# OlegArenz/gmmvi

Measured on AMD Instinct MI355X. Metric: samples_components_per_sec, higher is better.
Workload: dtype f32; 1 GPU; ns: stm target D=20, K=100 components (100/GPU), 100 samples/component, N=10000 samples/iter, SAMTRON (Stein, fixed K, reuse ratio 0, KL trust regions, improvement-based stepsizes); K=100, D=20, N=10000, parallelism=component-shard x1

## Files before the change

### gmmvi_amd/_lib.py

```python
import ctypes as C
import os

_HERE = os.path.dirname(os.path.abspath(__file__))
LIB_PATH = os.environ.get("GMMVI_HIP_LIB", os.path.join(_HERE, "libgmmvi_hip.so"))

GAUSS, STUDENT_T = 0, 1
SELF_NORMALIZED, OWN_SAMPLES_ONLY, EXPLICIT_ESTIMATE = 1, 2, 4
MAX_DIM = 64
MORE_REGISTER_MAX_DIM = 21
MORE_BLOCKED_MIN_DIM, MORE_BLOCKED_MAX_DIM = 64, 128
MAX_DIM_BLOCKED = 512
MAX_DIM_DIAG = 131072
BLOCKED_ABOVE_DEFAULT = 50


_blocked_above = None


def _atoi(text):
    import re
    m = re.match(r"\s*([+-]?\d+)", text)
    return int(m.group(1)) if m else 0


# ... 61 lines not shown
    "gmmvi_cholesky": (_i, [_p, _i, _i, _p, _p, _p]),
    "gmmvi_mixture_eval": (_i, [_p, _i, _f, _i, _i, _p, _p, _p, _i, _p, _p, _p]),
    "gmmvi_mixture_eval_dual": (_i, [_p, _i, _f, _i, _i, _p, _p, _p, _p, _i, _p, _p, _p, _p]),
    "gmmvi_target_planar": (_i, [_p, _i, _p, _i, _p, _f, _p, _i, _p, _p]),
    "gmmvi_target_logreg": (_i, [_p, _i, _i, _p, _f, _f, _p, _i, _p, _p]),
    "gmmvi_target_logreg_mb": (_i, [_p, _i, _i, _p, _i, _i, _u64, _u32, _f, _f, _p, _i, _p, _p]),
    "gmmvi_target_bnn": (_i, [_p, _i, _i, _i, _i, _p, _p, _u64, _u32, _i, _f, _f, _p, _i, _p, _p]),
    "gmmvi_bnn_predict": (_i, [_p, _i, _i, _i, _p, _i, _p, _i, _p]),
    "gmmvi_target_talos": (_i, [_p, _p, _p, _p, _i, _p, _p]),
    "gmmvi_talos_fk": (_i, [_p, _p, _p, _i, _p, _p]),
    "gmmvi_sample_components": (_i, [_p, _i, _i, _p, _p, _p, _i, _u64, _u64, _i, _p, _p, _p]),
    "gmmvi_philox_normals": (_i, [_p, _u64, _u64, _i, _i, _i, _p]),
    "gmmvi_philox_uniforms": (_i, [_p, _u64, _u64, _i, _i, _p]),
    "gmmvi_stein": (_i, [_p, _i, _i, _p, _p, _i, _p, _p, _p, _p, _p, _i, _i, _p, _p]),
    "gmmvi_more": (_i, [_p, _i, _i, _p, _p, _p, _i, _p, _p, _p, _p, _p, _i, _i, _p, _p, _p]),
    "gmmvi_more_blocked": (_i, [_p, _i, _i, _p, _p, _p, _i, _p, _p, _p, _p, _p, _i, _i, _p, _p, _p]),
    "gmmvi_update_components_kl": (_i, [_p, _i, _i, _p, _p, _p, _p, _p, _f, _f, _p, _p, _p, _p, _p, _p, _p]),
    "gmmvi_update_components_kl_reference": (_i, [_p, _i, _i, _p, _p, _p, _p, _p, _f, _f, _p, _p, _p, _p, _p, _p]),
    "gmmvi_update_components_direct": (_i, [_p, _i, _i, _p, _p, _p, _p, _p, _f, _p, _p, _p]),
    "gmmvi_update_components_iblr": (_i, [_p, _i, _i, _p, _p, _p, _p, _p, _f, _p, _p, _p]),
    "gmmvi_expected_log_ratios": (_i, [_p, _i, _i, _p, _p, _p, _p, _f, _p, _i, _p, _p, _p]),
    "gmmvi_update_weights_kl": (_i, [_p, _i, _p, _p, _p, _f, _p]),
    "gmmvi_update_weights_direct": (_i, [_p, _i, _p, _p, _p, _f]),
    "gmmvi_component_stepsize_improvement": (_i, [_p, _i, _p, _p, _p, _f, _f, _f, _f]),
    "gmmvi_weight_stepsize_improvement": (_i, [_p, _i, _p, _p, _p, _f, _f, _f, _f]),
    "gmmvi_train_iter_samtron": (_i, [_p, _p]),
    "gmmvi_sharded_scratch_floats": (_sz, [_i, _i, _i]),
    "gmmvi_train_iter_sharded_phase": (_i, [_p, _p, _i]),
    "gmmvi_comm_unique_id": (_i, [C.c_char_p]),
    "gmmvi_comm_init": (_i, [_p, C.c_char_p, _i, _i]),
    "gmmvi_comm_destroy": (_i, [_p]),
    "gmmvi_allgather_f32": (_i, [_p, _p, _p, _sz]),
    "gmmvi_allreduce_f32": (_i, [_p, _p, _sz, _i]),
    "gmmvi_combine_partials": (_i, [_p, _i, _i, _i, _p, _p, _p, _p]),
    "gmmvi_diag_packed_stride": (_sz, [_i]),
    "gmmvi_diag_pack": (_i, [_p, _i, _i, _p, _p, _p]),
    "gmmvi_diag_mixture_eval": (_i, [_p, _i, _i, _p, _p, _p, _p, _i, _p, _p, _p, _p]),
    "gmmvi_diag_sample": (_i, [_p, _i, _i, _p, _p, _p, _i, _u64, _u64, _i, _p, _p, _p]),
    "gmmvi_diag_stein": (_i, [_p, _i, _i, _p, _p, _i, _p, _p, _p, _p, _p, _i, _i, _p, _p]),
    "gmmvi_diag_embed": (_i, [_p, _i, _i, _p, _p]),
    "gmmvi_diag_extract": (_i, [_p, _i, _i, _p, _p]),
    "gmmvi_reciprocal_f32": (_i, [_p, _p, _sz, _p]),
    "gmmvi_update_components_diag_kl": (_i, [_p, _i, _i, _p, _p, _p, _p, _p, _f, _f, _p, _p, _p, _p, _p, _p]),
    "gmmvi_update_components_diag_iblr": (_i, [_p, _i, _i, _p, _p, _p, _p, _p, _f, _p, _p, _p]),
    "gmmvi_mmd_scratch_doubles": (_sz, [_i, _i]),
    "gmmvi_mmd_pair_sum": (_i, [_p, _p, _i, _p, _i, _i, _p, _p, _p]),
# ... 31 lines not shown
```

### gmmvi_amd/csrc/api.hip

```cpp
#include "common.h"
#include <cstring>
#include "blocked.h"

std::string g_gmmvi_global_err;

int gmmvi_ws_reserve(gmmvi_ctx* ctx, size_t nbytes) {
    ++ctx->ws_epoch;
    if (nbytes <= ctx->ws_bytes) return GMMVI_OK;
    GMMVI_HIP_CHECK(ctx, hipStreamSynchronize(ctx->stream));
    if (ctx->ws) GMMVI_HIP_CHECK(ctx, hipFree(ctx->ws));
    ctx->ws = nullptr;
    ctx->ws_bytes = 0;
    size_t want = nbytes + nbytes / 2;
    GMMVI_HIP_CHECK(ctx, hipMalloc(&ctx->ws, want));
    ctx->ws_bytes = want;
    return GMMVI_OK;
}

extern "C" {

int gmmvi_device_count(void) {
    int n = 0;
    if (hipGetDeviceCount(&n) != hipSuccess) return 0;
    return n;
}

int gmmvi_ctx_create(gmmvi_ctx** out, int device) {
    if (!out) return gmmvi_fail(nullptr, GMMVI_ERR_ARG, "gmmvi_ctx_create: out is NULL");
    *out = nullptr;
    int n = 0;
    hipError_t e = hipGetDeviceCount(&n);
    if (e != hipSuccess || n == 0)
        return gmmvi_fail(nullptr, GMMVI_ERR_HIP, std::string("no HIP device: ") + hipGetErrorString(e));
    if (device < 0 || device >= n) return gmmvi_fail(nullptr, GMMVI_ERR_ARG, "device index out of range");
    gmmvi_ctx* ctx = new gmmvi_ctx();
    ctx->device = device;
    e = hipSetDevice(device);
    if (e == hipSuccess) e = hipStreamCreateWithFlags(&ctx->stream, hipStreamNonBlocking);
    if (e != hipSuccess) {
        g_gmmvi_global_err = std::string("gmmvi_ctx_create: ") + hipGetErrorString(e);
        delete ctx;
        return GMMVI_ERR_HIP;
    }
    hipDeviceProp_t prop;
    if (hipGetDeviceProperties(&prop, device) == hipSuccess) ctx->num_cus = prop.multiProcessorCount;
    *out = ctx;
    return GMMVI_OK;
}

void gmmvi_ctx_destroy(gmmvi_ctx* ctx) {
    if (!ctx) return;
    gmmvi_comm_destroy(ctx);
    if (ctx->stream) {
        (void)hipStreamSynchronize(ctx->stream);
        (void)hipStreamDestroy(ctx->stream);
    }
    if (ctx->ws) (void)hipFree(ctx->ws);
    if (ctx->arena) (void)hipFree(ctx->arena);
    if (ctx->bimg) (void)hipFree(ctx->bimg);
    if (ctx->up_ring) {
        for (int i = 0; i < gmmvi_ctx::UP_SLOTS; ++i) (void)hipEventDestroy(ctx->up_event[i]);
        (void)hipHostFree(ctx->up_ring);
    }
    if (ctx->defer_ws) (void)hipFree(ctx->defer_ws);
    delete ctx;
}

const char* gmmvi_last_error(gmmvi_ctx* ctx) { return ctx ? ctx->err.c_str() : g_gmmvi_global_err.c_str(); }

int gmmvi_sync(gmmvi_ctx* ctx) {
    GMMVI_HIP_CHECK(ctx, hipStreamSynchronize(ctx->stream));
    return GMMVI_OK;
}

int gmmvi_malloc(gmmvi_ctx* ctx, size_t nbytes, void** out_dev) {
    GMMVI_ARG_CHECK(ctx, out_dev != nullptr);
    *out_dev = nullptr;
    if (nbytes == 0) nbytes = 4;
    GMMVI_HIP_CHECK(ctx, hipSetDevice(ctx->device));
    GMMVI_HIP_CHECK(ctx, hipMalloc(out_dev, nbytes));
    return GMMVI_OK;
}

int gmmvi_free(gmmvi_ctx* ctx, void* dev) {
    if (!dev) return GMMVI_OK;
    GMMVI_HIP_CHECK(ctx, hipFree(dev));
    return GMMVI_OK;
// ... 488 lines not shown
```

### gmmvi_amd/csrc/common.h

```cpp
#pragma once
#include <hip/hip_runtime.h>
#include <cstdio>
#include <cstring>
#include <cstdint>
#include <string>
#include <vector>
#include "../../include/gmmvi_hip.h"
#include "iter_prep.h"

struct CombineJob {
    int R = 0, N = 0, D = 0;
    long part_stride = 0;
    int first_block = 0, blocks = 0;
    const float* lp_parts = nullptr;
    const float* grad_parts = nullptr;
    const float* lp2_parts = nullptr;
    float* lp_out = nullptr;
    float* grad_out = nullptr;
    float* lp2_out = nullptr;
};

struct SampleJob {
    int K = 0, D = 0, uniform_count = 0;
    const float* means = nullptr; const float* chols = nullptr; const int32_t* offsets = nullptr;
// ... 14 lines not shown
}

struct gmmvi_ctx {
    int device = 0;
    hipStream_t stream = nullptr;
    std::string err;
    void* ws = nullptr;
    size_t ws_bytes = 0;
    uint64_t ws_epoch = 0;
    void* arena = nullptr;
    size_t arena_bytes = 0;
    static constexpr int UP_SLOTS = 64;
    static constexpr size_t UP_SLOT_BYTES = 64 * 1024;
    unsigned char* up_ring = nullptr;
    hipEvent_t up_event[UP_SLOTS] = {};
    bool up_used[UP_SLOTS] = {};
    int up_next = 0;
    void* bimg = nullptr;
    size_t bimg_bytes = 0;
    bool defer_combine = false;
    CombineJob pending;
    Riders riders;
    void* defer_ws = nullptr;
    size_t defer_bytes = 0;
    void* comm = nullptr;
    int n_ranks = 1, rank = 0;
    int num_cus = 256;
    unsigned func_attr_done = 0;
    bool prof = false;
    const char* prof_tag = nullptr;
    struct ProfRec { const char* name; hipEvent_t start, stop; double units; };
    std::vector<ProfRec> prof_recs;
};

struct GmmviProfScope {
    gmmvi_ctx* ctx; hipEvent_t stop = nullptr;
    GmmviProfScope(gmmvi_ctx* c, const char* name, double units = 0.0) : ctx(c) {
        if (!c->prof) return;
        hipEvent_t start;
        if (hipEventCreate(&start) != hipSuccess || hipEventCreate(&stop) != hipSuccess) { stop = nullptr; return; }
        (void)hipEventRecord(start, c->stream);
        c->prof_recs.push_back({name, start, stop, units});
    }
    ~GmmviProfScope() { if (stop) (void)hipEventRecord(stop, ctx->stream); }
};
#define GMMVI_PROF(ctx, name) GmmviProfScope prof_scope__(ctx, name)
// ... 33 lines not shown
int gmmvi_sample_components_prep(gmmvi_ctx* ctx, int K, int D, const float* means_dev, const float* chols_dev,
                                 const int32_t* offsets_dev, int N, int max_per_component, uint64_t seed, uint64_t first_index,
                                 float* X_out_dev, int32_t* mapping_out_dev, int32_t mapping_base, const PrepArgs& prep);
int gmmvi_combine_partials_internal(gmmvi_ctx* ctx, int R, int N, int D, const float* lp_parts_dev,
                                    const float* grad_parts_dev, float* lp_out_dev, float* grad_out_dev,
                                    const float* lp2_parts_dev, float* lp2_out_dev, long part_stride = 0);
int gmmvi_defer_reserve(gmmvi_ctx* ctx, size_t nbytes);
int gmmvi_flush_pending_combine(gmmvi_ctx* ctx);
CombineJob gmmvi_take_pending_combine(gmmvi_ctx* ctx, int threads, int first_block, bool light = false);
Riders gmmvi_take_pending_riders(gmmvi_ctx* ctx, int first_block, int threads, bool prep_only = false);
int gmmvi_flush_pending_riders(gmmvi_ctx* ctx);
struct SteinSlab;
int gmmvi_stein_partials(gmmvi_ctx* ctx, int K, int D, const float* packed_dev, const float* X_dev, int N, const float* ld_dev,
                         const float* qgrad_dev, const float* bg_dev, const float* tgrad_dev, int flags, SteinSlab* slab);
int gmmvi_stein_finalize_slab(gmmvi_ctx* ctx, int K, int D, const SteinSlab& slab, int N, int flags, const float* packed_dev,
                              float* H_neg_out_dev, float* g_neg_out_dev);
int gmmvi_update_components_kl_from_slab(gmmvi_ctx* ctx, int K, int D, const SteinSlab& slab, int N, int stein_flags,
                                         const float* packed_old_dev, float* H_neg_dev, float* g_neg_dev, float* means_dev,
                                         float* chols_dev, const float* stepsizes_dev, float temperature, float l2_init,
                                         float* last_eta_dev, float* l2_dev, float* num_received_updates_dev,
                                         int32_t* success_out_dev, float* packed_out_dev);
int gmmvi_update_weights_internal(gmmvi_ctx* ctx, int mode, int K, float* logw_dev, const float* E_dev,
                                  const float* stepsize_dev, float beta, float* kl_eta_out_dev, float* exp_out_dev);

inline int gmmvi_padded_dim(int D) {
    static const int dps[] = {2, 4, 8, 10, 12, 16, 20, 24, 32, 40, 50, 64};
    for (int dp : dps) if (D <= dp) return dp;
    return -1;
}

#define GMMVI_DISPATCH_DP(DPVAL, ...)                  \
    switch (DPVAL) {                                   \
        case 2:  { constexpr int DP = 2;  __VA_ARGS__; } break;  \
        case 4:  { constexpr int DP = 4;  __VA_ARGS__; } break;  \
        case 8:  { constexpr int DP = 8;  __VA_ARGS__; } break;  \
        case 10: { constexpr int DP = 10; __VA_ARGS__; } break;  \
        case 12: { constexpr int DP = 12; __VA_ARGS__; } break;  \
        case 16: { constexpr int DP = 16; __VA_ARGS__; } break;  \
        case 20: { constexpr int DP = 20; __VA_ARGS__; } break;  \
        case 24: { constexpr int DP = 24; __VA_ARGS__; } break;  \
        case 32: { constexpr int DP = 32; __VA_ARGS__; } break;  \
        case 40: { constexpr int DP = 40; __VA_ARGS__; } break;  \
        case 50: { constexpr int DP = 50; __VA_ARGS__; } break;  \
        case 64: { constexpr int DP = 64; __VA_ARGS__; } break;  \
        default: return gmmvi_fail(ctx, GMMVI_ERR_ARG, "unsupported dimension (D must be <= 64)"); \
    }
// ... 95 lines not shown
```

### gmmvi_amd/csrc/fused.hip

```cpp
#include "common.h"
#include "stepsize_rules.h"
#include "iter_prep.h"
#include "stein_finalize.h"

namespace {
struct Arena {
    float *ld, *lq, *qgrad, *bg, *H, *g, *E;
    int32_t *mapping, *success;
};

}

static int arena_reserve(gmmvi_ctx* ctx, size_t floats) {
    if (floats * sizeof(float) <= ctx->arena_bytes) return GMMVI_OK;
    GMMVI_HIP_CHECK(ctx, hipStreamSynchronize(ctx->stream));
    if (ctx->arena) GMMVI_HIP_CHECK(ctx, hipFree(ctx->arena));
    ctx->arena = nullptr;
    ctx->arena_bytes = 0;
    size_t want = floats * sizeof(float) * 3 / 2;
    GMMVI_HIP_CHECK(ctx, hipMalloc(&ctx->arena, want));
    ctx->arena_bytes = want;
    return GMMVI_OK;
}

#define GMMVI_TRY(call)                \
    do {                               \
        int rc__ = (call);             \
        if (rc__ != GMMVI_OK) return rc__; \
    } while (0)

static int train_iter_samtron_body(gmmvi_ctx* ctx, const gmmvi_samtron_plan* p);

extern "C" int gmmvi_train_iter_samtron(gmmvi_ctx* ctx, const gmmvi_samtron_plan* p) {
    GMMVI_ARG_CHECK(ctx, ctx != nullptr);
    int rc = gmmvi_flush_pending_combine(ctx);
    if (rc == GMMVI_OK) rc = train_iter_samtron_body(ctx, p);
    if (rc != GMMVI_OK) {
        ctx->pending = CombineJob();
        ctx->riders.prep_blocks = ctx->riders.sample_blocks = 0;
        ctx->defer_combine = false;
        ctx->prof_tag = nullptr;
    }
    return rc;
}

static int train_iter_samtron_body(gmmvi_ctx* ctx, const gmmvi_samtron_plan* p) {
    GMMVI_ARG_CHECK(ctx, p != nullptr);
    GMMVI_ARG_CHECK(ctx, (p->target_kind >= 0 && p->target_kind <= 2) || p->target_kind == 4);
    GMMVI_ARG_CHECK(ctx, p->target_kind != 2 || (p->logreg_A && p->logreg_M >= 1 && p->logreg_prior_std > 0.f));
    GMMVI_ARG_CHECK(ctx, p->target_kind != 4 || (p->talos_model && p->talos_context && p->D == 34));
    const int K = p->K, D = p->D, N = p->N;
    GMMVI_ARG_CHECK(ctx, K >= 1 && D >= 1 && D < GMMVI_MAX_DIM && N >= 1);
    GMMVI_ARG_CHECK(ctx, p->means && p->chols && p->logw && p->packed && p->packed_new && p->stepsizes && p->last_eta &&
                             p->l2 && p->num_updates && p->offsets && p->bg_logw && p->db_samples && p->db_tlp &&
                             p->db_tgrad && p->db_mapping && p->reward_next && p->wstate);
    GMMVI_ARG_CHECK(ctx, p->n_old >= 0 && p->max_per_component >= 0 && p->phase >= 0 && p->phase <= 2);
    GMMVI_ARG_CHECK(ctx, p->n_old == 0 || (p->bg_packed != nullptr && p->bg_K >= 1 && p->bg_old != nullptr && p->bg_logw_new != nullptr));
    const int n_old = p->n_old;
    const int Na = n_old + N;
    const size_t KN = (size_t)K * Na, ND = (size_t)Na * D;
    const size_t floats = KN + 4 * (size_t)Na + ND + (size_t)K * D * D + (size_t)K * D + 3 * (size_t)K + Na + 64;
    GMMVI_TRY(arena_reserve(ctx, floats));
    Arena a;
    float* base = (float*)ctx->arena;
// ... 87 lines not shown
    GMMVI_TRY(gmmvi_flush_pending_riders(ctx));
    SteinSlab slab{nullptr, nullptr, 0};
    GMMVI_TRY(gmmvi_stein_partials(ctx, K, D, p->packed, xa, Na, a.ld, a.qgrad, a.bg, tgrad_a, p->stein_flags, &slab));
    GMMVI_TRY(gmmvi_update_components_kl_from_slab(ctx, K, D, slab, Na, p->stein_flags, p->packed, a.H, a.g, p->means, p->chols,
                                                   p->stepsizes, p->temperature, p->l2_init, p->last_eta, p->l2, p->num_updates,
                                                   p->success_out ? p->success_out : a.success, p->packed_new));
    }
    if (phase == 1) return GMMVI_OK;
    ctx->defer_combine = true;
    ctx->prof_tag = "sweep_post";
    int rc_post = gmmvi_mixture_eval(ctx, GMMVI_GAUSS, 0.f, K, D, p->packed_new, p->logw, xa, Na, a.ld, a.lq, nullptr);
    ctx->defer_combine = false;
    ctx->prof_tag = nullptr;
    GMMVI_TRY(rc_post);
    if (p->presample_next && n_old == 0) {
        const int max_pc = p->max_per_component > 0 ? p->max_per_component : (N + K - 1) / K;
        SampleJob& sj = ctx->riders.sample;
        sj.K = K; sj.D = D; sj.uniform_count = (long)K * max_pc == N ? max_pc : 0;
        sj.means = p->means; sj.chols = p->chols; sj.offsets = p->offsets;
        sj.seed = p->seed; sj.first_index = p->first_index + (uint64_t)N;
        sj.X = x + (size_t)N * D; sj.mapping = p->db_mapping + N; sj.mapping_base = p->mapping_base + K;
        ctx->riders.sample_blocks = K * ((max_pc + 255) / 256);
    }
    GMMVI_TRY(gmmvi_expected_log_ratios(ctx, K, Na, a.ld, a.bg, tlp_a, a.lq, p->temperature, p->logw,
                                        (p->stein_flags & GMMVI_SELF_NORMALIZED) ? 1 : 0, a.E, p->reward_next, nullptr));
    GMMVI_TRY(gmmvi_flush_pending_riders(ctx));
    if (K > 1) {
        GMMVI_TRY(gmmvi_update_weights_internal(ctx, p->weight_update_mode == 0 ? 0 : 1, K, p->logw, a.E, p->wstate,
                                                p->temperature, nullptr, p->weight_slot));
    }
    return GMMVI_OK;
}


namespace {
struct ShardArena { float *ld, *lq, *bg, *qgrad, *H, *g, *E; int32_t* success; };
}
extern "C" size_t gmmvi_sharded_scratch_floats(int K, int D, int N) {
    if (K < 1 || D < 1 || N < 1) return 0;
    return (size_t)K * N + 2 * (size_t)N + (size_t)N * D + (size_t)K * D * D + (size_t)K * D + 2 * (size_t)K + 64;
}
static void shard_arena(float* base, int K, int D, int N, ShardArena& a) {
    a.ld = base; base += (size_t)K * N;
    a.lq = base; base += N;
    a.bg = base; base += N;
    a.qgrad = base; base += (size_t)N * D;
    a.H = base; base += (size_t)K * D * D;
    a.g = base; base += (size_t)K * D;
    a.E = base; base += K;
    a.success = (int32_t*)base;
}

static int sharded_phase_body(gmmvi_ctx* ctx, const gmmvi_sharded_plan* p, int phase) {
// ... 133 lines not shown
```

### gmmvi_amd/csrc/weights.hip

```cpp
#include "common.h"
#include "riders.h"
#include "stepsize_rules.h"
#include "wave_reduce.h"
#include "combine.h"
#include <cfloat>

namespace {

__device__ __forceinline__ float wsum(float v) { return gmmvi_wave_sum(v); }
__device__ __forceinline__ float wmax(float v) { return gmmvi_wave_max(v); }

__device__ float block_max(float v, float* red) {
    v = wmax(v);
    __syncthreads();
    if ((threadIdx.x & 63) == 0) red[threadIdx.x >> 6] = v;
    __syncthreads();
    return fmaxf(fmaxf(red[0], red[1]), fmaxf(red[2], red[3]));
}
__device__ float block_sum(float v, float* red) {
    v = wsum(v);
    __syncthreads();
    if ((threadIdx.x & 63) == 0) red[threadIdx.x >> 6] = v;
    __syncthreads();
    return (red[0] + red[1]) + (red[2] + red[3]);
}

template <int R>
// ... 8 lines not shown
            const int n = min(n0 + 1024 * u, N - 1);
            av[u] = row[n] - bg[n];
            float lq;
            if constexpr (R == 0) lq = logq[n];
            else if constexpr (R > 0) lq = combine_log_values_n<R>(logq, N, n);
            else lq = combine_log_values(logq, Rrt, N, n);
            rv[u] = tlp[n] - beta * lq;
        }
#pragma unroll
        for (int u = 0; u < B; ++u) {
            if (n0 + 1024 * u < N) {
                const float a = av[u], rho = rv[u];
                const float mn = fmaxf(m, a);
                const float sc = __expf(m - mn), e = __expf(a - mn);
                s = fmaf(s, sc, e);
                se = fmaf(se, sc, e * rho);
                s2 = fmaf(s2, sc * sc, e * e);
                m = mn;
            }
        }
    }
}

__device__ __forceinline__ void elr_body(int N, const float* __restrict__ ld, const float* __restrict__ bg,
                                         const float* __restrict__ tlp, const float* __restrict__ logq, int logq_R,
                                         float beta, const float* __restrict__ logw, int self_normalized,
                                         float* __restrict__ E_out, float* __restrict__ reward_out,
                                         float* __restrict__ ess_out) {
    __shared__ float red[4][16];
    const int k = blockIdx.x;
    const float* row = ld + (size_t)k * N;
    float m = -3.0e38f, s = 0.f, se = 0.f, s2 = 0.f;
    switch (logq_R) {
        case 0: elr_accumulate<0>(N, row, bg, tlp, logq, 0, beta, m, s, se, s2); break;
        case 2: elr_accumulate<2>(N, row, bg, tlp, logq, 2, beta, m, s, se, s2); break;
        case 3: elr_accumulate<3>(N, row, bg, tlp, logq, 3, beta, m, s, se, s2); break;
        case 4: elr_accumulate<4>(N, row, bg, tlp, logq, 4, beta, m, s, se, s2); break;
        case 5: elr_accumulate<5>(N, row, bg, tlp, logq, 5, beta, m, s, se, s2); break;
        case 6: elr_accumulate<6>(N, row, bg, tlp, logq, 6, beta, m, s, se, s2); break;
        case 7: elr_accumulate<7>(N, row, bg, tlp, logq, 7, beta, m, s, se, s2); break;
        case 8: elr_accumulate<8>(N, row, bg, tlp, logq, 8, beta, m, s, se, s2); break;
        case 10: elr_accumulate<10>(N, row, bg, tlp, logq, 10, beta, m, s, se, s2); break;
        case 12: elr_accumulate<12>(N, row, bg, tlp, logq, 12, beta, m, s, se, s2); break;
        case 16: elr_accumulate<16>(N, row, bg, tlp, logq, 16, beta, m, s, se, s2); break;
        default: elr_accumulate<-1>(N, row, bg, tlp, logq, logq_R, beta, m, s, se, s2); break;
    }
    const float mw = wmax(m);
    const float f = __expf(m - mw);
    s = wsum(s * f); se = wsum(se * f); s2 = wsum(s2 * f * f);
    const int lane = threadIdx.x & 63, wave = threadIdx.x >> 6;
    if (lane == 0) { red[0][wave] = mw; red[1][wave] = s; red[2][wave] = se; red[3][wave] = s2; }
    __syncthreads();
    if (threadIdx.x == 0) {
        float M = -3.0e38f;
        for (int w = 0; w < 16; ++w) M = fmaxf(M, red[0][w]);
        float S = 0.f, SE = 0.f, S2 = 0.f;
        for (int w = 0; w < 16; ++w) {
            const float g = __expf(red[0][w] - M);
            S = fmaf(red[1][w], g, S); SE = fmaf(red[2][w], g, SE); S2 = fmaf(red[3][w], g * g, S2);
        }
        const float E = self_normalized ? SE / S : SE * __expf(M) / (float)N;
        if (E_out) E_out[k] = E;
        if (reward_out) reward_out[k] = beta * logw[k] + E;
        if (ess_out) ess_out[k] = (S * S) / S2;
    }
}

__global__ __launch_bounds__(1024) void elr_kernel(int N, const float* __restrict__ ld, const float* __restrict__ bg,
                                                   const float* __restrict__ tlp, const float* __restrict__ logq, int logq_R,
                                                   float beta, const float* __restrict__ logw, int self_normalized,
                                                   float* __restrict__ E_out, float* __restrict__ reward_out,
                                                   float* __restrict__ ess_out) {
    elr_body(N, ld, bg, tlp, logq, logq_R, beta, logw, self_normalized, E_out, reward_out, ess_out);
}

template <int DP>
__global__ __launch_bounds__(1024) void elr_riders_kernel(int N, const float* __restrict__ ld, const float* __restrict__ bg,
                                                          const float* __restrict__ tlp, const float* __restrict__ logq,
                                                          int logq_R, float beta, const float* __restrict__ logw,
                                                          int self_normalized, float* __restrict__ E_out,
                                                          float* __restrict__ reward_out, float* __restrict__ ess_out,
                                                          Riders riders) {
    extern __shared__ __align__(16) float sm_riders[];
    if (riders_carried<DP>(riders, sm_riders)) return;
    elr_body(N, ld, bg, tlp, logq, logq_R, beta, logw, self_normalized, E_out, reward_out, ess_out);
}

__device__ float wave_lse(const float* v, int K) {
// ... 77 lines not shown
    bool ub_ok = false;
    for (int it = 0; it < 50; ++it) {
        eta = expf(log_eta);
        if (fabsf(expf(ub) - expf(lb)) < 1e-1f) break;
        kl = weights_kl_reg<NE>(eta, beta, lw, E, h, v);
        if (fabsf(bound - kl) < 1e-1f * bound) { lb = ub; break; }
        if (bound > kl) { ub = log_eta; ub_ok = true; } else { lb = log_eta; }
        log_eta = 0.5f * (ub + lb);
    }
    if (lb == ub) {
    } else if (ub_ok) {
        eta = expf(ub);
        kl = weights_kl_reg<NE>(eta, beta, lw, E, h, v);
    } else {
        updated = false;
        kl = -1.f; eta = -1.f;
    }
#pragma unroll
    for (int e = 0; e < NE; ++e)
        if (h[e]) nl[t + 64 * e] = v[e];
    __syncthreads();
}

__global__ __launch_bounds__(64) void update_weights_kernel(int mode, int K, float* __restrict__ logw,
                                                            const float* __restrict__ E_in, const float* __restrict__ stepsize,
                                                            float beta, float* __restrict__ kl_eta_out,
                                                            float* __restrict__ exp_out) {
    extern __shared__ float sm[];
    float* lw = sm; float* E = sm + K; float* nl = sm + 2 * K;
    const int t = threadIdx.x;
    for (int i = t; i < K; i += 64) { lw[i] = logw[i]; E[i] = E_in[i]; nl[i] = logw[i]; }
    __syncthreads();
    if (K <= 1) return;
    const float bound = stepsize[0];
    float kl = -1.f, eta = -1.f;
    bool updated = true;
    if (mode == 1) {
        for (int i = t; i < K; i += 64) nl[i] = lw[i] + bound / beta * E[i];
        __syncthreads();
        float l = wave_lse(nl, K);
        for (int i = t; i < K; i += 64) nl[i] = fmaxf(nl[i] - l, -69.07f);
        __syncthreads();
        l = wave_lse(nl, K);
        for (int i = t; i < K; i += 64) nl[i] -= l;
        __syncthreads();
    } else {
        if (K <= 128) {
            weights_search_reg<2>(K, beta, bound, lw, E, nl, kl, eta, updated);
        } else if (K <= 256) {
            weights_search_reg<4>(K, beta, bound, lw, E, nl, kl, eta, updated);
        } else if (K <= 512) {
            weights_search_reg<8>(K, beta, bound, lw, E, nl, kl, eta, updated);
        } else if (K <= 1024) {
            weights_search_reg<16>(K, beta, bound, lw, E, nl, kl, eta, updated);
// ... 12 lines not shown
            if (lb == ub) {
            } else if (ub_ok) {
                eta = expf(ub);
                kl = weights_kl(eta, beta, lw, E, nl, K);
            } else {
                updated = false;
                kl = -1.f; eta = -1.f;
            }
        }
    }
    if (!updated) {
        for (int i = t; i < K; i += 64) nl[i] = lw[i];
        __syncthreads();
    }
    const float l = wave_lse(nl, K);
    for (int i = t; i < K; i += 64) {
        const float v = nl[i] - l;
        logw[i] = v;
        if (exp_out) exp_out[i] = expf(v);
    }
    if (t == 0 && kl_eta_out) { kl_eta_out[0] = kl; kl_eta_out[1] = eta; }
}

__global__ void component_stepsize_kernel(int K, float* __restrict__ stepsizes, const float* __restrict__ prev,
                                          const float* __restrict__ last, float mn, float mx, float inc, float dec) {
    const int k = blockIdx.x * blockDim.x + threadIdx.x;
    if (k >= K) return;
    stepsizes[k] = component_stepsize_rule(stepsizes[k], prev[k], last[k], mn, mx, inc, dec);
}

__global__ __launch_bounds__(64) void weight_stepsize_kernel(int K, const float* __restrict__ logw,
                                                             const float* __restrict__ rewards_last, float* __restrict__ state,
                                                             float mn, float mx, float inc, float dec) {
    weight_stepsize_wave(K, logw, rewards_last, state, mn, mx, inc, dec, threadIdx.x);
}

}

extern "C" {

int gmmvi_expected_log_ratios(gmmvi_ctx* ctx, int K, int N, const float* ld_dev, const float* bg_dev,
                              const float* tlp_dev, const float* logq_dev, float beta, const float* logw_dev,
                              int self_normalized, float* E_out_dev, float* reward_out_dev, float* ess_out_dev) {
    GMMVI_ARG_CHECK(ctx, K >= 1 && N >= 1);
    GMMVI_ARG_CHECK(ctx, ld_dev && bg_dev && tlp_dev && logq_dev && logw_dev);
    int logq_R = 0;
    {
        const CombineJob& j = ctx->pending;
        if (j.R > 0 && j.lp_out == logq_dev && j.N == N && !j.grad_out && !j.lp2_out) {
            logq_R = j.R;
            logq_dev = j.lp_parts;
            ctx->pending = CombineJob();
        } else {
            int rc = gmmvi_flush_pending_combine(ctx);
            if (rc != GMMVI_OK) return rc;
        }
    }
    GMMVI_PROF(ctx, "expected_log_ratios");
    const Riders riders = gmmvi_take_pending_riders(ctx, K, 1024);
    if (riders.prep_blocks + riders.sample_blocks > 0) {
        const int dp = gmmvi_padded_dim(riders.sample_blocks > 0 ? riders.sample.D : 2);
        GMMVI_DISPATCH_DP(dp, hipLaunchKernelGGL((elr_riders_kernel<DP>), dim3(K + riders.prep_blocks + riders.sample_blocks),
                                                 dim3(1024), riders_lds_bytes(riders), ctx->stream, N, ld_dev, bg_dev, tlp_dev,
                                                 logq_dev, logq_R, beta, logw_dev, self_normalized, E_out_dev, reward_out_dev,
                                                 ess_out_dev, riders));
    } else {
        hipLaunchKernelGGL(elr_kernel, dim3(K), dim3(1024), 0, ctx->stream, N, ld_dev, bg_dev, tlp_dev, logq_dev, logq_R, beta,
                           logw_dev, self_normalized, E_out_dev, reward_out_dev, ess_out_dev);
    }
    GMMVI_LAUNCH_CHECK(ctx);
    return GMMVI_OK;
}

}

int gmmvi_update_weights_internal(gmmvi_ctx* ctx, int mode, int K, float* logw_dev, const float* E_dev,
                                  const float* stepsize_dev, float beta, float* kl_eta_out_dev, float* exp_out_dev) {
    GMMVI_ARG_CHECK(ctx, K >= 1 && K <= 4096);
    GMMVI_ARG_CHECK(ctx, logw_dev && E_dev && stepsize_dev);
    GMMVI_PROF(ctx, "update_weights");
    hipLaunchKernelGGL(update_weights_kernel, dim3(1), dim3(64), (size_t)3 * K * sizeof(float), ctx->stream, mode, K,
                       logw_dev, E_dev, stepsize_dev, beta, kl_eta_out_dev, exp_out_dev);
    GMMVI_LAUNCH_CHECK(ctx);
    return GMMVI_OK;
}

extern "C" {

int gmmvi_update_weights_kl(gmmvi_ctx* ctx, int K, float* logw_dev, const float* E_dev, const float* stepsize_dev,
                            float beta, float* kl_eta_out_dev) {
    return gmmvi_update_weights_internal(ctx, 0, K, logw_dev, E_dev, stepsize_dev, beta, kl_eta_out_dev, nullptr);
}

int gmmvi_update_weights_direct(gmmvi_ctx* ctx, int K, float* logw_dev, const float* E_dev,
                                const float* stepsize_dev, float beta) {
    return gmmvi_update_weights_internal(ctx, 1, K, logw_dev, E_dev, stepsize_dev, beta, nullptr, nullptr);
}

int gmmvi_component_stepsize_improvement(gmmvi_ctx* ctx, int K, float* stepsizes_dev, const float* rewards_prev_dev,
                                         const float* rewards_last_dev, float min_stepsize, float max_stepsize,
                                         float inc_factor, float dec_factor) {
    GMMVI_ARG_CHECK(ctx, K >= 1 && stepsizes_dev && rewards_prev_dev && rewards_last_dev);
    GMMVI_PROF(ctx, "component_stepsize");
    hipLaunchKernelGGL(component_stepsize_kernel, dim3((K + 127) / 128), dim3(128), 0, ctx->stream, K, stepsizes_dev,
                       rewards_prev_dev, rewards_last_dev, min_stepsize, max_stepsize, inc_factor, dec_factor);
    GMMVI_LAUNCH_CHECK(ctx);
    return GMMVI_OK;
}

int gmmvi_weight_stepsize_improvement(gmmvi_ctx* ctx, int K, const float* logw_dev, const float* rewards_last_dev,
// ... 12 lines not shown
```

### gmmvi_amd/hip_ops.py

```python
import math

import numpy as np

from . import _lib
from .device import DeviceArray

F32, I32 = np.dtype(np.float32), np.dtype(np.int32)


def _req(a, shape, dtype=F32, name="array"):
    if not isinstance(a, DeviceArray):
        raise TypeError(f"{name}: expected DeviceArray, got {type(a)}")
    if a.dtype != dtype or tuple(a.shape) != tuple(shape):
        raise ValueError(f"{name}: expected {dtype}{tuple(shape)}, got {a.dtype}{a.shape}")
    return a.ptr


def _opt(a, shape, dtype=F32, name="array"):
    return None if a is None else _req(a, shape, dtype, name)


def packed_stride(d):
    s = int(_lib.load().gmmvi_packed_stride(int(d)))
    if s == 0:
# ... 415 lines not shown
    if reward_out is not None:
        _req(reward_out, (k,), name="reward_out")
    e = ctx.empty((k,))
    ess = ctx.empty((k,)) if want_ess else None
    ctx.check(ctx.lib.gmmvi_expected_log_ratios(ctx.handle, k, n, ld.ptr, bg.ptr, tlp.ptr, logq.ptr, float(beta),
                                                logw.ptr, 1 if self_normalized else 0, e.ptr,
                                                None if reward_out is None else reward_out.ptr,
                                                None if ess is None else ess.ptr))
    return e, ess


def update_weights(ctx, mode, logw, e, stepsize, beta, want_info=False):
    k = logw.shape[0]
    _req(logw, (k,), name="logw"); _req(e, (k,), name="E"); _req(stepsize, (1,), name="stepsize")
    info = ctx.empty((2,)) if (want_info and mode == "trust-region") else None
    if mode == "trust-region":
        ctx.check(ctx.lib.gmmvi_update_weights_kl(ctx.handle, k, logw.ptr, e.ptr, stepsize.ptr, float(beta),
                                                  None if info is None else info.ptr))
    else:
        ctx.check(ctx.lib.gmmvi_update_weights_direct(ctx.handle, k, logw.ptr, e.ptr, stepsize.ptr, float(beta)))
    return info


def component_stepsize_improvement(ctx, stepsizes, prev, last, mn, mx, inc, dec):
    k = stepsizes.shape[0]
    _req(stepsizes, (k,), name="stepsizes"); _req(prev, (k,), name="prev"); _req(last, (k,), name="last")
    ctx.check(ctx.lib.gmmvi_component_stepsize_improvement(ctx.handle, k, stepsizes.ptr, prev.ptr, last.ptr, float(mn),
                                                           float(mx), float(inc), float(dec)))


def weight_stepsize_improvement(ctx, logw, rewards_last, state, mn, mx, inc, dec):
    k = logw.shape[0]
    _req(logw, (k,), name="logw"); _req(rewards_last, (k,), name="rewards_last"); _req(state, (2,), name="state")
    ctx.check(ctx.lib.gmmvi_weight_stepsize_improvement(ctx.handle, k, logw.ptr, rewards_last.ptr, state.ptr, float(mn),
                                                        float(mx), float(inc), float(dec)))


def combine_partials(ctx, lp_parts, grad_parts, d):
    r, n = lp_parts.shape
    _req(lp_parts, (r, n), name="lp_parts")
    if grad_parts is not None:
        _req(grad_parts, (r, n, d), name="grad_parts")
    lp = ctx.empty((n,))
    grad = ctx.empty((n, d)) if grad_parts is not None else None
    ctx.check(ctx.lib.gmmvi_combine_partials(ctx.handle, r, n, d, lp_parts.ptr,
                                             None if grad_parts is None else grad_parts.ptr, lp.ptr,
# ... 91 lines not shown
```

### include/gmmvi_hip.h

```cpp
#ifndef GMMVI_HIP_H
#define GMMVI_HIP_H

#include <stddef.h>
#include <stdint.h>

#ifdef __cplusplus
extern "C" {
#endif

typedef struct gmmvi_ctx gmmvi_ctx;

enum gmmvi_status {
    GMMVI_OK = 0,
    GMMVI_ERR_HIP = -1,
    GMMVI_ERR_ARG = -2,
    GMMVI_ERR_RCCL = -3,
    GMMVI_ERR_STATE = -4
};

enum gmmvi_family {
    GMMVI_GAUSS = 0,
    GMMVI_STUDENT_T = 1
};

// ... 117 lines not shown
                               float* num_received_updates_dev, int32_t* success_out_dev, float* kl_out_dev,
                               int32_t* n_probes_out_dev, float* packed_out_dev);
int gmmvi_update_components_kl_reference(gmmvi_ctx* ctx, int K, int D, float* means_dev, float* chols_dev,
                                         const float* H_neg_dev, const float* g_neg_dev, const float* stepsizes_dev,
                                         float temperature, float l2_init, float* last_eta_dev, float* l2_dev,
                                         float* num_received_updates_dev, int32_t* success_out_dev, float* kl_out_dev,
                                         int32_t* n_probes_out_dev);
int gmmvi_update_components_direct(gmmvi_ctx* ctx, int K, int D, float* means_dev, float* chols_dev,
                                   const float* H_neg_dev, const float* g_neg_dev, const float* stepsizes_dev,
                                   float l2_init, float* l2_dev, float* num_received_updates_dev,
                                   int32_t* success_out_dev);
int gmmvi_update_components_iblr(gmmvi_ctx* ctx, int K, int D, float* means_dev, float* chols_dev,
                                 const float* H_neg_dev, const float* g_neg_dev, const float* stepsizes_dev,
                                 float l2_init, float* l2_dev, float* num_received_updates_dev,
                                 int32_t* success_out_dev);

int gmmvi_expected_log_ratios(gmmvi_ctx* ctx, int K, int N, const float* ld_dev, const float* bg_dev,
                              const float* tlp_dev, const float* logq_dev, float beta, const float* logw_dev,
                              int self_normalized, float* E_out_dev, float* reward_out_dev, float* ess_out_dev);
int gmmvi_update_weights_kl(gmmvi_ctx* ctx, int K, float* logw_dev, const float* E_dev, const float* stepsize_dev,
                            float beta, float* kl_eta_out_dev);
int gmmvi_update_weights_direct(gmmvi_ctx* ctx, int K, float* logw_dev, const float* E_dev,
                                const float* stepsize_dev, float beta);
int gmmvi_component_stepsize_improvement(gmmvi_ctx* ctx, int K, float* stepsizes_dev, const float* rewards_prev_dev,
                                         const float* rewards_last_dev, float min_stepsize, float max_stepsize,
                                         float inc_factor, float dec_factor);
int gmmvi_weight_stepsize_improvement(gmmvi_ctx* ctx, int K, const float* logw_dev, const float* rewards_last_dev,
                                      float* state_dev, float min_stepsize, float max_stepsize, float inc_factor,
                                      float dec_factor);

typedef struct gmmvi_samtron_plan {
    int32_t K, D, N;
    int32_t target_kind;
    int32_t target_family, target_K;
    float target_nu;
    const float* target_packed;
    const float* target_logw;
    const float* planar_prior_std;
    const float* planar_goals;
    int32_t planar_goals_count;
    float planar_likelihood_std;
    float* means; float* chols; float* logw;
    const float* packed;
    float* packed_new;
    float* stepsizes; float* last_eta; float* l2; float* num_updates;
    int32_t* success_out;
// ... 113 lines not shown
```

Measured before the change: 5.137 billion samples*components/s.

## Fuse expected-log-ratio and weight-update kernels via last-block ticket handoff

The expected-log-ratios kernel and the weight-update kernel now run as one launch. Each block atomically publishes its E and reward values and draws a ticket. The block that draws the last ticket resets the counter and runs the weight update in its first wave. This removes one kernel launch and the gap between the two kernels in each SAMTRON iteration. In exchange it adds atomics, a per-context ticket buffer and a serial tail in a single block, and it falls back to the old two-kernel path when prep riders are pending or LDS would be too large.

```diff
diff --git a/gmmvi_amd/_lib.py b/gmmvi_amd/_lib.py
--- a/gmmvi_amd/_lib.py
+++ b/gmmvi_amd/_lib.py
@@ -107,6 +107,8 @@
     "gmmvi_expected_log_ratios": (_i, [_p, _i, _i, _p, _p, _p, _p, _f, _p, _i, _p, _p, _p]),
     "gmmvi_update_weights_kl": (_i, [_p, _i, _p, _p, _p, _f, _p]),
     "gmmvi_update_weights_direct": (_i, [_p, _i, _p, _p, _p, _f]),
+    "gmmvi_expected_log_ratios_update_weights": (_i, [_p, _i, _i, _p, _p, _p, _p, _f, _p, _i, _p, _p, _i, _p, _p, _p, _i, _p, _p,
+                                                      _p, _i, _i, _u64, _u64, _p, _p]),
     "gmmvi_component_stepsize_improvement": (_i, [_p, _i, _p, _p, _p, _f, _f, _f, _f]),
     "gmmvi_weight_stepsize_improvement": (_i, [_p, _i, _p, _p, _p, _f, _f, _f, _f]),
     "gmmvi_train_iter_samtron": (_i, [_p, _p]),
diff --git a/gmmvi_amd/csrc/api.hip b/gmmvi_amd/csrc/api.hip
--- a/gmmvi_amd/csrc/api.hip
+++ b/gmmvi_amd/csrc/api.hip
@@ -37,7 +37,11 @@
     ctx->device = device;
     e = hipSetDevice(device);
     if (e == hipSuccess) e = hipStreamCreateWithFlags(&ctx->stream, hipStreamNonBlocking);
+    if (e == hipSuccess) e = hipMalloc((void**)&ctx->tickets, gmmvi_ctx::TICKET_BYTES);
+    if (e == hipSuccess) e = hipMemset(ctx->tickets, 0, gmmvi_ctx::TICKET_BYTES);
     if (e != hipSuccess) {
+        if (ctx->tickets) (void)hipFree(ctx->tickets);
+        if (ctx->stream) (void)hipStreamDestroy(ctx->stream);
         g_gmmvi_global_err = std::string("gmmvi_ctx_create: ") + hipGetErrorString(e);
         delete ctx;
         return GMMVI_ERR_HIP;
@@ -63,6 +67,7 @@
         (void)hipHostFree(ctx->up_ring);
     }
     if (ctx->defer_ws) (void)hipFree(ctx->defer_ws);
+    if (ctx->tickets) (void)hipFree(ctx->tickets);
     delete ctx;
 }
 
diff --git a/gmmvi_amd/csrc/common.h b/gmmvi_amd/csrc/common.h
--- a/gmmvi_amd/csrc/common.h
+++ b/gmmvi_amd/csrc/common.h
@@ -60,6 +60,8 @@
     CombineJob pending;
     Riders riders;
     void* defer_ws = nullptr;
+    unsigned* tickets = nullptr;
+    static constexpr size_t TICKET_BYTES = 64;
     size_t defer_bytes = 0;
     void* comm = nullptr;
     int n_ranks = 1, rank = 0;
@@ -139,6 +141,10 @@
                                          int32_t* success_out_dev, float* packed_out_dev);
 int gmmvi_update_weights_internal(gmmvi_ctx* ctx, int mode, int K, float* logw_dev, const float* E_dev,
                                   const float* stepsize_dev, float beta, float* kl_eta_out_dev, float* exp_out_dev);
+int gmmvi_elr_update_weights_internal(gmmvi_ctx* ctx, int K, int N, const float* ld_dev, const float* bg_dev, const float* tlp_dev,
+                                      const float* logq_dev, float beta, float* logw_dev, int self_normalized, float* E_out_dev,
+                                      float* reward_out_dev, int mode, const float* stepsize_dev, float* kl_eta_out_dev,
+                                      float* exp_out_dev);
 
 inline int gmmvi_padded_dim(int D) {
     static const int dps[] = {2, 4, 8, 10, 12, 16, 20, 24, 32, 40, 50, 64};
diff --git a/gmmvi_amd/csrc/fused.hip b/gmmvi_amd/csrc/fused.hip
--- a/gmmvi_amd/csrc/fused.hip
+++ b/gmmvi_amd/csrc/fused.hip
@@ -40,6 +40,7 @@
         ctx->riders.prep_blocks = ctx->riders.sample_blocks = 0;
         ctx->defer_combine = false;
         ctx->prof_tag = nullptr;
+        if (ctx->tickets) (void)hipMemsetAsync(ctx->tickets, 0, gmmvi_ctx::TICKET_BYTES, ctx->stream);
     }
     return rc;
 }
@@ -173,13 +174,10 @@
         sj.X = x + (size_t)N * D; sj.mapping = p->db_mapping + N; sj.mapping_base = p->mapping_base + K;
         ctx->riders.sample_blocks = K * ((max_pc + 255) / 256);
     }
-    GMMVI_TRY(gmmvi_expected_log_ratios(ctx, K, Na, a.ld, a.bg, tlp_a, a.lq, p->temperature, p->logw,
-                                        (p->stein_flags & GMMVI_SELF_NORMALIZED) ? 1 : 0, a.E, p->reward_next, nullptr));
+    GMMVI_TRY(gmmvi_elr_update_weights_internal(ctx, K, Na, a.ld, a.bg, tlp_a, a.lq, p->temperature, p->logw,
+                                                (p->stein_flags & GMMVI_SELF_NORMALIZED) ? 1 : 0, a.E, p->reward_next,
+                                                p->weight_update_mode == 0 ? 0 : 1, p->wstate, nullptr, p->weight_slot));
     GMMVI_TRY(gmmvi_flush_pending_riders(ctx));
-    if (K > 1) {
-        GMMVI_TRY(gmmvi_update_weights_internal(ctx, p->weight_update_mode == 0 ? 0 : 1, K, p->logw, a.E, p->wstate,
-                                                p->temperature, nullptr, p->weight_slot));
-    }
     return GMMVI_OK;
 }
 
diff --git a/gmmvi_amd/csrc/weights.hip b/gmmvi_amd/csrc/weights.hip
--- a/gmmvi_amd/csrc/weights.hip
+++ b/gmmvi_amd/csrc/weights.hip
@@ -3,6 +3,7 @@
 #include "stepsize_rules.h"
 #include "wave_reduce.h"
 #include "combine.h"
+#include <algorithm>
 #include <cfloat>
 
 namespace {
@@ -57,11 +58,11 @@
     }
 }
 
-__device__ __forceinline__ void elr_body(int N, const float* __restrict__ ld, const float* __restrict__ bg,
+template <bool PUBLISH = false>
+__device__ __forceinline__ bool elr_body(int N, const float* __restrict__ ld, const float* __restrict__ bg,
                                          const float* __restrict__ tlp, const float* __restrict__ logq, int logq_R,
-                                         float beta, const float* __restrict__ logw, int self_normalized,
-                                         float* __restrict__ E_out, float* __restrict__ reward_out,
-                                         float* __restrict__ ess_out) {
+                                         float beta, const float* logw, int self_normalized, float* E_out, float* reward_out,
+                                         float* __restrict__ ess_out, unsigned* ticket = nullptr, int K = 0) {
     __shared__ float red[4][16];
     const int k = blockIdx.x;
     const float* row = ld + (size_t)k * N;
@@ -95,10 +96,24 @@
             S = fmaf(red[1][w], g, S); SE = fmaf(red[2][w], g, SE); S2 = fmaf(red[3][w], g * g, S2);
         }
         const float E = self_normalized ? SE / S : SE * __expf(M) / (float)N;
-        if (E_out) E_out[k] = E;
-        if (reward_out) reward_out[k] = beta * logw[k] + E;
+        if constexpr (PUBLISH) {
+            __hip_atomic_store(E_out + k, E, __ATOMIC_RELAXED, __HIP_MEMORY_SCOPE_AGENT);
+            if (reward_out)
+                __hip_atomic_store(reward_out + k, beta * logw[k] + E, __ATOMIC_RELAXED, __HIP_MEMORY_SCOPE_AGENT);
+            asm volatile("s_waitcnt vmcnt(0)" ::: "memory");
+            const unsigned drawn = __hip_atomic_fetch_add(ticket, 1u, __ATOMIC_RELAXED, __HIP_MEMORY_SCOPE_AGENT);
+            red[0][0] = drawn == (unsigned)(K - 1) ? 1.f : 0.f;
+        } else {
+            if (E_out) E_out[k] = E;
+            if (reward_out) reward_out[k] = beta * logw[k] + E;
+        }
         if (ess_out) ess_out[k] = (S * S) / S2;
     }
+    if constexpr (PUBLISH) {
+        __syncthreads();
+        return red[0][0] != 0.f;
+    }
+    return false;
 }
 
 __global__ __launch_bounds__(1024) void elr_kernel(int N, const float* __restrict__ ld, const float* __restrict__ bg,
@@ -222,14 +237,17 @@
     __syncthreads();
 }
 
-__global__ __launch_bounds__(64) void update_weights_kernel(int mode, int K, float* __restrict__ logw,
-                                                            const float* __restrict__ E_in, const float* __restrict__ stepsize,
-                                                            float beta, float* __restrict__ kl_eta_out,
-                                                            float* __restrict__ exp_out) {
-    extern __shared__ float sm[];
+template <bool HANDED_OVER>
+__device__ __forceinline__ void update_weights_body(int mode, int K, float* logw, const float* E_in, const float* stepsize,
+                                                    float beta, float* kl_eta_out, float* exp_out, float* sm) {
     float* lw = sm; float* E = sm + K; float* nl = sm + 2 * K;
     const int t = threadIdx.x;
-    for (int i = t; i < K; i += 64) { lw[i] = logw[i]; E[i] = E_in[i]; nl[i] = logw[i]; }
+    for (int i = t; i < K; i += 64) {
+        float e;
+        if constexpr (HANDED_OVER) e = __hip_atomic_load(E_in + i, __ATOMIC_RELAXED, __HIP_MEMORY_SCOPE_AGENT);
+        else e = E_in[i];
+        lw[i] = logw[i]; E[i] = e; nl[i] = logw[i];
+    }
     __syncthreads();
     if (K <= 1) return;
     const float bound = stepsize[0];
@@ -288,6 +306,36 @@
     if (t == 0 && kl_eta_out) { kl_eta_out[0] = kl; kl_eta_out[1] = eta; }
 }
 
+__global__ __launch_bounds__(64) void update_weights_kernel(int mode, int K, float* __restrict__ logw,
+                                                            const float* __restrict__ E_in, const float* __restrict__ stepsize,
+                                                            float beta, float* __restrict__ kl_eta_out,
+                                                            float* __restrict__ exp_out) {
+    extern __shared__ float sm[];
+    update_weights_body<false>(mode, K, logw, E_in, stepsize, beta, kl_eta_out, exp_out, sm);
+}
+
+struct WeightEpilogue {
+    int mode, K;
+    float* logw; float* E;
+    const float* stepsize;
+    float* kl_eta_out; float* exp_out;
+    unsigned* ticket;
+};
+
+template <int DP>
+__global__ __launch_bounds__(1024) void elr_update_weights_kernel(int N, const float* __restrict__ ld, const float* __restrict__ bg,
+                                                                  const float* __restrict__ tlp, const float* __restrict__ logq,
+                                                                  int logq_R, float beta, int self_normalized, float* reward_out,
+                                                                  WeightEpilogue w, Riders riders) {
+    extern __shared__ __align__(16) float sm_riders[];
+    if (riders_carried<DP>(riders, sm_riders)) return;
+    const bool last = elr_body<true>(N, ld, bg, tlp, logq, logq_R, beta, w.logw, self_normalized, w.E, reward_out, nullptr,
+                                     w.ticket, w.K);
+    if (!last || threadIdx.x >= 64) return;
+    if (threadIdx.x == 0) __hip_atomic_store(w.ticket, 0u, __ATOMIC_RELAXED, __HIP_MEMORY_SCOPE_AGENT);
+    update_weights_body<true>(w.mode, w.K, w.logw, w.E, w.stepsize, beta, w.kl_eta_out, w.exp_out, sm_riders);
+}
+
 __global__ void component_stepsize_kernel(int K, float* __restrict__ stepsizes, const float* __restrict__ prev,
                                           const float* __restrict__ last, float mn, float mx, float inc, float dec) {
     const int k = blockIdx.x * blockDim.x + threadIdx.x;
@@ -301,6 +349,17 @@
     weight_stepsize_wave(K, logw, rewards_last, state, mn, mx, inc, dec, threadIdx.x);
 }
 
+}
+
+static int elr_take_merge(gmmvi_ctx* ctx, int N, const float*& logq_dev, int& logq_R) {
+    const CombineJob& j = ctx->pending;
+    if (j.R > 0 && j.lp_out == logq_dev && j.N == N && !j.grad_out && !j.lp2_out) {
+        logq_R = j.R;
+        logq_dev = j.lp_parts;
+        ctx->pending = CombineJob();
+        return GMMVI_OK;
+    }
+    return gmmvi_flush_pending_combine(ctx);
 }
 
 extern "C" {
@@ -311,17 +370,8 @@
     GMMVI_ARG_CHECK(ctx, K >= 1 && N >= 1);
     GMMVI_ARG_CHECK(ctx, ld_dev && bg_dev && tlp_dev && logq_dev && logw_dev);
     int logq_R = 0;
-    {
-        const CombineJob& j = ctx->pending;
-        if (j.R > 0 && j.lp_out == logq_dev && j.N == N && !j.grad_out && !j.lp2_out) {
-            logq_R = j.R;
-            logq_dev = j.lp_parts;
-            ctx->pending = CombineJob();
-        } else {
-            int rc = gmmvi_flush_pending_combine(ctx);
-            if (rc != GMMVI_OK) return rc;
-        }
-    }
+    int rc_merge = elr_take_merge(ctx, N, logq_dev, logq_R);
+    if (rc_merge != GMMVI_OK) return rc_merge;
     GMMVI_PROF(ctx, "expected_log_ratios");
     const Riders riders = gmmvi_take_pending_riders(ctx, K, 1024);
     if (riders.prep_blocks + riders.sample_blocks > 0) {
@@ -351,7 +401,63 @@
     return GMMVI_OK;
 }
 
+int gmmvi_elr_update_weights_internal(gmmvi_ctx* ctx, int K, int N, const float* ld_dev, const float* bg_dev, const float* tlp_dev,
+                                      const float* logq_dev, float beta, float* logw_dev, int self_normalized, float* E_out_dev,
+                                      float* reward_out_dev, int mode, const float* stepsize_dev, float* kl_eta_out_dev,
+                                      float* exp_out_dev) {
+    GMMVI_ARG_CHECK(ctx, K >= 1 && N >= 1);
+    GMMVI_ARG_CHECK(ctx, ld_dev && bg_dev && tlp_dev && logq_dev && logw_dev && E_out_dev && stepsize_dev);
+    const size_t lds = std::max(riders_lds_bytes(ctx->riders), (size_t)3 * K * sizeof(float));
+    if (K < 2 || K > 4096 || ctx->riders.prep_blocks > 0 || lds > 64 * 1024 || !ctx->tickets) {
+        int rc = gmmvi_expected_log_ratios(ctx, K, N, ld_dev, bg_dev, tlp_dev, logq_dev, beta, logw_dev, self_normalized, E_out_dev,
+                                           reward_out_dev, nullptr);
+        if (rc == GMMVI_OK) rc = gmmvi_flush_pending_riders(ctx);
+        if (rc == GMMVI_OK && K > 1)
+            rc = gmmvi_update_weights_internal(ctx, mode, K, logw_dev, E_out_dev, stepsize_dev, beta, kl_eta_out_dev, exp_out_dev);
+        return rc;
+    }
+    int logq_R = 0;
+    int rc_merge = elr_take_merge(ctx, N, logq_dev, logq_R);
+    if (rc_merge != GMMVI_OK) return rc_merge;
+    GMMVI_PROF(ctx, "expected_log_ratios");
+    const Riders riders = gmmvi_take_pending_riders(ctx, K, 1024);
+    const WeightEpilogue w{mode, K, logw_dev, E_out_dev, stepsize_dev, kl_eta_out_dev, exp_out_dev, ctx->tickets};
+    const int dp = gmmvi_padded_dim(riders.sample_blocks > 0 ? riders.sample.D : 2);
+    GMMVI_DISPATCH_DP(dp, hipLaunchKernelGGL((elr_update_weights_kernel<DP>), dim3(K + riders.sample_blocks), dim3(1024), lds,
+                                             ctx->stream, N, ld_dev, bg_dev, tlp_dev, logq_dev, logq_R, beta, self_normalized,
+                                             reward_out_dev, w, riders));
+    GMMVI_LAUNCH_CHECK(ctx);
+    return GMMVI_OK;
+}
+
 extern "C" {
+
+int gmmvi_expected_log_ratios_update_weights(gmmvi_ctx* ctx, int K, int N, const float* ld_dev, const float* bg_dev,
+                                             const float* tlp_dev, const float* logq_dev, float beta, float* logw_dev,
+                                             int self_normalized, float* E_out_dev, float* reward_out_dev, int direct,
+                                             const float* stepsize_dev, float* kl_eta_out_dev, float* exp_out_dev, int draw_D,
+                                             const float* means_dev, const float* chols_dev, const int32_t* offsets_dev,
+                                             int draw_N, int max_per_component, uint64_t seed, uint64_t first_index,
+                                             float* X_out_dev, int32_t* mapping_out_dev) {
+    GMMVI_ARG_CHECK(ctx, ctx != nullptr && K >= 1);
+    GMMVI_ARG_CHECK(ctx, (ctx->riders.prep_blocks | ctx->riders.sample_blocks) == 0);
+    if (draw_D > 0) {
+        GMMVI_ARG_CHECK(ctx, draw_D < GMMVI_MAX_DIM && gmmvi_padded_dim(draw_D) > 0 && means_dev && chols_dev && offsets_dev &&
+                                 X_out_dev && draw_N >= 1 && max_per_component >= 1);
+        SampleJob& sj = ctx->riders.sample;
+        sj.K = K; sj.D = draw_D; sj.uniform_count = (long)K * max_per_component == draw_N ? max_per_component : 0;
+        sj.means = means_dev; sj.chols = chols_dev; sj.offsets = offsets_dev;
+        sj.seed = seed; sj.first_index = first_index;
+        sj.X = X_out_dev; sj.mapping = mapping_out_dev; sj.mapping_base = 0;
+        ctx->riders.sample_blocks = K * ((max_per_component + 255) / 256);
+    }
+    int rc = gmmvi_elr_update_weights_internal(ctx, K, N, ld_dev, bg_dev, tlp_dev, logq_dev, beta, logw_dev, self_normalized,
+                                               E_out_dev, reward_out_dev, direct ? 1 : 0, stepsize_dev, direct ? nullptr : kl_eta_out_dev,
+                                               exp_out_dev);
+    if (rc == GMMVI_OK) rc = gmmvi_flush_pending_riders(ctx);
+    if (rc != GMMVI_OK) ctx->riders.prep_blocks = ctx->riders.sample_blocks = 0;
+    return rc;
+}
 
 int gmmvi_update_weights_kl(gmmvi_ctx* ctx, int K, float* logw_dev, const float* E_dev, const float* stepsize_dev,
                             float beta, float* kl_eta_out_dev) {
diff --git a/gmmvi_amd/hip_ops.py b/gmmvi_amd/hip_ops.py
--- a/gmmvi_amd/hip_ops.py
+++ b/gmmvi_amd/hip_ops.py
@@ -461,6 +461,34 @@
     return info
 
 
+def expected_log_ratios_update_weights(ctx, mode, ld, bg, tlp, logq, beta, logw, stepsize, self_normalized=True, reward_out=None,
+                                       want_info=False, exp_out=None, draw=None):
+    k, n = ld.shape
+    _req(ld, (k, n), name="ld"); _req(bg, (n,), name="bg"); _req(tlp, (n,), name="tlp"); _req(logq, (n,), name="logq")
+    _req(logw, (k,), name="logw"); _req(stepsize, (1,), name="stepsize")
+    if reward_out is not None:
+        _req(reward_out, (k,), name="reward_out")
+    if exp_out is not None:
+        _req(exp_out, (k,), name="exp_out")
+    e = ctx.empty((k,))
+    info = ctx.empty((2,)) if (want_info and mode == "trust-region") else None
+    x = mapping = None
+    dargs = [0, None, None, None, 0, 0, 0, 0, None, None]
+    if draw is not None:
+        means, chols, offsets = draw["means"], draw["chols"], draw["offsets"]
+        d = means.shape[1]
+        _req(means, (k, d), name="means"); _req(chols, (k, d, d), name="chols"); _req(offsets, (k + 1,), I32, name="offsets")
+        x = ctx.empty((int(draw["n"]), d))
+        mapping = ctx.empty((int(draw["n"]),), I32)
+        dargs = [d, means.ptr, chols.ptr, offsets.ptr, int(draw["n"]), int(draw["max_per_component"]), int(draw.get("seed", 0)),
+                 int(draw.get("first_index", 0)), x.ptr, mapping.ptr]
+    ctx.check(ctx.lib.gmmvi_expected_log_ratios_update_weights(
+        ctx.handle, k, n, ld.ptr, bg.ptr, tlp.ptr, logq.ptr, float(beta), logw.ptr, 1 if self_normalized else 0, e.ptr,
+        None if reward_out is None else reward_out.ptr, 0 if mode == "trust-region" else 1, stepsize.ptr,
+        None if info is None else info.ptr, None if exp_out is None else exp_out.ptr, *dargs))
+    return e, info, x, mapping
+
+
 def component_stepsize_improvement(ctx, stepsizes, prev, last, mn, mx, inc, dec):
     k = stepsizes.shape[0]
     _req(stepsizes, (k,), name="stepsizes"); _req(prev, (k,), name="prev"); _req(last, (k,), name="last")
diff --git a/include/gmmvi_hip.h b/include/gmmvi_hip.h
--- a/include/gmmvi_hip.h
+++ b/include/gmmvi_hip.h
@@ -163,6 +163,13 @@
                             float beta, float* kl_eta_out_dev);
 int gmmvi_update_weights_direct(gmmvi_ctx* ctx, int K, float* logw_dev, const float* E_dev,
                                 const float* stepsize_dev, float beta);
+int gmmvi_expected_log_ratios_update_weights(gmmvi_ctx* ctx, int K, int N, const float* ld_dev, const float* bg_dev,
+                                             const float* tlp_dev, const float* logq_dev, float beta, float* logw_dev,
+                                             int self_normalized, float* E_out_dev, float* reward_out_dev, int direct,
+                                             const float* stepsize_dev, float* kl_eta_out_dev, float* exp_out_dev, int draw_D,
+                                             const float* means_dev, const float* chols_dev, const int32_t* offsets_dev,
+                                             int draw_N, int max_per_component, uint64_t seed, uint64_t first_index,
+                                             float* X_out_dev, int32_t* mapping_out_dev);
 int gmmvi_component_stepsize_improvement(gmmvi_ctx* ctx, int K, float* stepsizes_dev, const float* rewards_prev_dev,
                                          const float* rewards_last_dev, float min_stepsize, float max_stepsize,
                                          float inc_factor, float dec_factor);
```

Result: no change. 5.093 billion samples*components/s (-0.9%).
